# FaspDevTeam/faspsolver

Measured on AMD Instinct MI355X. Metric: AMG-PCG solve DOF/s (3D 7-pt Poisson 256^3, classical AMG V(1,1) w-Jacobi + PCG, rtol 1e-8), higher is better.
Workload: dtype f64

## Files before the change

### faspsolver_amd/__init__.py

```python
import ctypes as C
import os
import subprocess

import numpy as np

from . import _types as T
from ._types import *

_HERE = os.path.dirname(os.path.abspath(__file__))
LIB_PATH = os.environ.get("FASP_HIP_LIB") or os.path.join(_HERE, "libfasp_hip.so")
_lib = None

EXPORTS = [
    "fasp_param_amg_init", "fasp_param_solver_init", "fasp_solver_dcsr_krylov_amg",
    "fasp_blas_dcsr_mxv", "fasp_blas_dcsr_aAxpy", "fasp_blas_darray_dotprod",
    "fasp_blas_darray_norm2", "fasp_blas_darray_norminf", "fasp_blas_darray_axpy",
    "fasp_blas_darray_axpby", "fasp_smoother_dcsr_jacobi",
    "fasp_blas_dbsr_mxv", "fasp_blas_dbsr_aAxpy", "fasp_dbsr_getdiaginv", "fasp_smoother_dbsr_jacobi1",
    "fasp_solver_dbsr_pcg", "fasp_solver_dbsr_pbcgs", "fasp_solver_dbsr_pgmres", "fasp_solver_dbsr_pvgmres",
    "fasp_solver_dbsr_pvfgmres", "fasp_hip_bsr_precond_setup", "fasp_hip_bsr_precond_fct", "fasp_hip_bsr_precond_free",
    "fasp_hip_param_input", "fasp_fwrapper_dcsr_krylov_amg_", "fasp_dcsrvec_read2", "fasp_dvec_read",
    "fasp_dbsr_read", "fasp_dcoo_read", "fasp_dcoo_read1", "fasp_dcoo_shift_read", "fasp_dmtx_read", "fasp_dmtxsym_read", "fasp_dvec_write", "fasp_dcsr_write_coo", "fasp_dcsrvec_write2", "fasp_fwrapper_dcsr_amg_", "fasp_fwrapper_dbsr_krylov_amg_", "fasp_hip_free_bsr", "fasp_hip_comm_selftest", "fasp_hip_amg_kernel_info", "fasp_hip_coarse_kernel_info", "fasp_hip_bsr_coarse_kernel_info", "fasp_hip_coding_selftest", "fasp_solver_amg", "fasp_solver_famg", "fasp_hip_amg_solve", "fasp_precond_diag", "fasp_precond_dbsr_diag", "fasp_solver_dcsr_itsolver", "fasp_solver_dcsr_krylov", "fasp_solver_dcsr_krylov_diag", "fasp_solver_dbsr_itsolver", "fasp_solver_dbsr_krylov", "fasp_solver_dbsr_krylov_diag", "fasp_hip_mxv_csr", "fasp_hip_mxv_bsr", "fasp_solver_matfree_init", "fasp_solver_pcg", "fasp_solver_pbcgs", "fasp_solver_pgcg", "fasp_solver_pminres", "fasp_solver_pgmres", "fasp_solver_pvgmres", "fasp_solver_pvfgmres", "fasp_solver_itsolver", "fasp_solver_krylov", "fasp_solver_dcsr_pcg", "fasp_solver_dcsr_pminres", "fasp_solver_dcsr_pgcg", "fasp_solver_dcsr_pgcr", "fasp_solver_dcsr_pbcgs", "fasp_solver_dcsr_pgmres", "fasp_solver_dcsr_pvgmres",
    "fasp_solver_dcsr_pvfgmres", "fasp_hip_precond_setup", "fasp_hip_precond_fct", "fasp_hip_precond_free",
    "fasp_hip_time_bsr_mxv", "fasp_solver_dbsr_krylov_amg", "fasp_hip_bsr_amg_create", "fasp_hip_bsr_amg_create_host",
# ... 1 lines not shown
    "fasp_hip_bsr_amg_get_diaginv", "fasp_hip_bsr_solve",
    "fasp_hip_set_device", "fasp_hip_device_count", "fasp_hip_device_identity", "fasp_hip_available",
    "fasp_hip_amg_create", "fasp_hip_amg_create_host", "fasp_hip_amg_upload",
    "fasp_hip_amg_destroy", "fasp_hip_amg_num_levels", "fasp_hip_amg_get_matrix",
    "fasp_hip_amg_get_cfmark", "fasp_hip_solve", "fasp_hip_set_rhs", "fasp_hip_set_guess",
    "fasp_hip_solve_resident", "fasp_hip_get_solution", "fasp_hip_device_synchronize",
    "fasp_hip_precond_amg",
    "fasp_hip_poisson7pt", "fasp_hip_aniso27pt", "fasp_hip_free_system", "fasp_hip_time_kernel", "fasp_hip_measure_ceilings", "fasp_hip_amg_publish", "fasp_hip_amg_attach", "fasp_hip_amg_unpublish",
    "fasp_precond_setup", "fasp_precond_amg", "fasp_precond_famg", "fasp_precond_amli", "fasp_precond_namli", "fasp_amg_data_create", "fasp_amg_data_free", "fasp_param_amg_to_prec", "fasp_param_prec_to_amg", "fasp_mem_free", "fasp_mem_calloc", "fasp_dvec_alloc", "fasp_dvec_set", "fasp_dvec_free", "fasp_dvec_create", "fasp_dcsr_create", "fasp_dcsr_free", "fasp_smoother_dcsr_gs", "fasp_smoother_dcsr_sor", "fasp_smoother_dcsr_L1diag",
    "fasp_hip_tune", "fasp_hip_comm_unique_id", "fasp_hip_comm_init", "fasp_hip_comm_finalize",
    "fasp_hip_comm_rank", "fasp_hip_comm_size", "fasp_hip_version", "fasp_hip_comm_init_shm",
    "fasp_hip_dist_plan", "fasp_hip_dist_level_info", "fasp_hip_dist_get_matrix",
    "fasp_hip_dist_get_list",
    "fasp_blas_dcsr_vmv", "fasp_blas_dcsr_mxv_agg", "fasp_blas_dcsr_aAxpy_agg", "fasp_blas_darray_ax",
    "fasp_blas_darray_axpyz", "fasp_blas_darray_norm1", "fasp_darray_cp", "fasp_darray_set", "fasp_dvec_isnan",
    "fasp_hip_time_matrix", "fasp_hip_bsr_dist_info", "fasp_hip_seq_schedule_selftest", "fasp_hip_seq_chain_selftest", "fasp_hip_cluster_order", "fasp_hip_permute_csr", "fasp_hip_comm_init_ipc", "fasp_hip_comm_stats", "fasp_hip_comm_timing", "fasp_hip_estream_selftest", "fasp_hip_sell_selftest", "fasp_hip_csr_plan", "fasp_hip_level_op", "fasp_hip_matrix_op", "fasp_hip_matrix_traits",
    "fasp_param_ilu_init", "fasp_ilu_data_create", "fasp_ilu_data_free", "fasp_mem_iludata_check", "fasp_ilu_dcsr_setup",
    "fasp_precond_ilu", "fasp_precond_ilu_forward", "fasp_precond_ilu_backward", "fasp_solver_dcsr_krylov_ilu",
    "fasp_solver_dcsr_krylov_ilu_M", "fasp_smoother_dcsr_ilu", "fasp_fwrapper_dcsr_krylov_ilu_",
    "fasp_hip_ilu_resident_count", "fasp_hip_ilu_time",
    "fasp_ilu_dbsr_setup", "fasp_precond_dbsr_ilu", "fasp_solver_dbsr_krylov_ilu", "fasp_smoother_dbsr_ilu",
    "fasp_fwrapper_dbsr_krylov_ilu_",
    "fasp_hip_bsr_amg_get_ilu", "fasp_hip_bsr_amg_ilu_info", "fasp_hip_bsr_amg_ilu_smooth_time",
    "fasp_hip_bsr_sweep", "fasp_hip_csr_sweep",
    "fasp_blas_dcsr_rap", "fasp_hip_dcsr_rap", "fasp_hip_rap_info", "fasp_hip_rap_device_count", "fasp_hip_rap_time",
    "fasp_dstr_create", "fasp_dstr_alloc", "fasp_dstr_free", "fasp_dstr_cp", "fasp_format_dstr_dcsr", "fasp_dstr_read",
    "fasp_blas_dstr_aAxpy", "fasp_blas_dstr_mxv", "fasp_precond_dstr_diag", "fasp_solver_dstr_pcg", "fasp_solver_dstr_pbcgs",
    "fasp_solver_dstr_pminres", "fasp_solver_dstr_pgmres", "fasp_solver_dstr_pvgmres", "fasp_solver_dstr_itsolver",
    "fasp_solver_dstr_krylov", "fasp_solver_dstr_krylov_diag", "fasp_hip_mxv_str", "fasp_hip_str_form", "fasp_hip_time_str_mxv",
    "fasp_ilu_dstr_setup0", "fasp_ilu_dstr_setup1", "fasp_precond_dstr_ilu0", "fasp_precond_dstr_ilu1", "fasp_solver_dstr_krylov_ilu",
    "fasp_hip_str_ilu_form", "fasp_hip_str_ilu_apply", "fasp_hip_time_str_ilu",
# ... 674 lines not shown
```

### faspsolver_amd/csrc/device_csr.hip.h

```cpp

struct DevCSR {
    int     row = 0, col = 0, nnz = 0;
    int*    ia  = nullptr;
    int*    ja  = nullptr;
    double* val = nullptr;
    int*    dpos = nullptr;
    bool    dup_diag = false;
    bool    sorted = false;
    int     lanes = 8;
    int     kind = 0;
    int     tile_rows = 256;
    int     wrows = 64, wcap = 512;
    unsigned char* code = nullptr;
    int*    rowbase = nullptr;
    int*    doff = nullptr;
    double* dval = nullptr;
    unsigned short* pat = nullptr;
    int*    pstart = nullptr;
    int*    plen = nullptr;
    int*    poff = nullptr;
    double* pval = nullptr;
    int     npat = 0, npent = 0;
    unsigned short* ja16 = nullptr;
    int*            jbase = nullptr;
// ... 5 lines not shown
    int*    tcols = nullptr;
    long long ntcols = 0;
    const int* bridge = nullptr;
    double*    bscratch = nullptr;
    int        bridge_dir = 0;
    int*       es_tab = nullptr;
    unsigned short* es_ja16 = nullptr;
    double*    es_part = nullptr;
    int        es_W = 0, es_nc = 0;
    unsigned*      sell_code = nullptr;
    int*           sell_meta = nullptr;
    unsigned char* sell_rlen = nullptr;
    double*        sell_tab = nullptr;
    int            sell_nv = 0, sell_obits = 0, sell_nslice = 0;
    long long      sell_slots = 0;
    void    release()
    {
        if (sell_code) (void)hipFree(sell_code);
        if (sell_meta) (void)hipFree(sell_meta);
        if (sell_rlen) (void)hipFree(sell_rlen);
        if (sell_tab) (void)hipFree(sell_tab);
        sell_code = nullptr; sell_meta = nullptr; sell_rlen = nullptr; sell_tab = nullptr; sell_nv = sell_obits = sell_nslice = 0; sell_slots = 0;
        if (es_tab) (void)hipFree(es_tab);
        if (es_part) (void)hipFree(es_part);
        if (es_ja16) (void)hipFree(es_ja16);
        es_tab = nullptr; es_part = nullptr; es_ja16 = nullptr; es_W = es_nc = 0;
        if (bscratch) (void)hipFree(bscratch);
        bscratch = nullptr; bridge = nullptr; bridge_dir = 0;
        if (lja16) (void)hipFree(lja16);
        if (tptr) (void)hipFree(tptr);
        if (tcols) (void)hipFree(tcols);
        lja16 = nullptr; tptr = nullptr; tcols = nullptr;
// ... 786 lines not shown
    std::vector<int> meta(2 * ns + 1);
    std::copy(S.sptr.begin(), S.sptr.end(), meta.begin());
    std::copy(S.sbase.begin(), S.sbase.end(), meta.begin() + (long)ns + 1);
    HIPCK(hipMalloc(&D.sell_code, sizeof(unsigned) * (size_t)std::max<long long>(S.slots, 1)));
    HIPCK(hipMalloc(&D.sell_meta, sizeof(int) * meta.size()));
    HIPCK(hipMalloc(&D.sell_rlen, (size_t)H.row));
    HIPCK(hipMalloc(&D.sell_tab, sizeof(double) * (size_t)S.nv));
    HIPCK(hipMemcpy(D.sell_code, S.code.data(), sizeof(unsigned) * (size_t)S.slots, hipMemcpyHostToDevice));
    HIPCK(hipMemcpy(D.sell_meta, meta.data(), sizeof(int) * meta.size(), hipMemcpyHostToDevice));
    HIPCK(hipMemcpy(D.sell_rlen, S.rlen.data(), (size_t)H.row, hipMemcpyHostToDevice));
    HIPCK(hipMemcpy(D.sell_tab, S.tab.data(), sizeof(double) * (size_t)S.nv, hipMemcpyHostToDevice));
    D.sell_nv = S.nv; D.sell_obits = S.obits; D.sell_nslice = S.nslice; D.sell_slots = S.slots;
    return FASP_SUCCESS;
}

static int upload_csr(const HostCSR& H, DevCSR& D)
{
    D.row = H.row; D.col = H.col; D.nnz = H.nnz;
    HIPCK(hipMalloc(&D.ia, sizeof(int) * ((size_t)H.row + 1)));
    HIPCK(hipMalloc(&D.ja, sizeof(int) * std::max<size_t>(H.nnz, 1)));
    HIPCK(hipMalloc(&D.val, sizeof(double) * (std::max<size_t>(H.nnz, 1) + 2)));
    HIPCK(hipMemsetAsync(D.val + std::max<size_t>(H.nnz, 1), 0, sizeof(double) * 2, g_ctx.stream));
    HIPCK(hipMemcpyAsync(D.ia, H.ia.data(), sizeof(int) * ((size_t)H.row + 1), hipMemcpyHostToDevice, g_ctx.stream));
    pick_kernel(D);
    auto upload_plain = [&]() -> int {
        HIPCK(hipMemcpyAsync(D.ja, H.ja.data(), sizeof(int) * (size_t)H.nnz, hipMemcpyHostToDevice, g_ctx.stream));
        HIPCK(hipMemcpyAsync(D.val, H.val.data(), sizeof(double) * (size_t)H.nnz, hipMemcpyHostToDevice, g_ctx.stream));
        return 0;
    };
    if (compress_enabled() && H.nnz >= 4096 && (double)H.nnz <= 48.0 * H.row) {
        Buf<unsigned short> pat; Buf<int> prb;
        std::vector<int> pstart, plen, poff; std::vector<double> pval;
        static const bool rowpat_on = !(std::getenv("FASP_HIP_ROWPAT") && std::atoi(std::getenv("FASP_HIP_ROWPAT")) == 0);
        if (rowpat_on && build_rowpat(H, pat, pstart, plen, poff, pval, prb)) {
            D.npat = (int)pstart.size(); D.npent = (int)poff.size();
            HIPCK(hipMalloc(&D.pat, sizeof(unsigned short) * ((size_t)H.row + 2)));
            HIPCK(hipMalloc(&D.pstart, sizeof(int) * pstart.size()));
            HIPCK(hipMalloc(&D.plen, sizeof(int) * plen.size()));
            HIPCK(hipMemcpy(D.plen, plen.data(), sizeof(int) * plen.size(), hipMemcpyHostToDevice));
// ... 101 lines not shown
        lap("row sort");
        HIPCK(hipMemcpy(D.ja, sj.data(), sizeof(int) * (size_t)H.nnz, hipMemcpyHostToDevice));
        HIPCK(hipMemcpy(D.val, sv.data(), sizeof(double) * (size_t)H.nnz, hipMemcpyHostToDevice));
        lap("memcpy");
        if (square && D.kind == 2) {
            HIPCK(hipMalloc(&D.dpos, sizeof(int) * (size_t)std::max(H.row, 1)));
            HIPCK(hipMemcpy(D.dpos, dp.data(), sizeof(int) * (size_t)H.row, hipMemcpyHostToDevice));
        }
        D.sorted = true;
        if (upload_ja16(D, H.ia.data(), sj.data()) < 0) return ERROR_ALLOC_MEM;
        return build_estream(H.ia.data(), H.row, H.nnz, D);
    }
    if (upload_plain() < 0) return ERROR_ALLOC_MEM;
    if (D.kind == 2 && !g_oneshot_upload && build_xtile(H, D) < 0) return ERROR_ALLOC_MEM;
    if (D.kind == 2 && compress_enabled() && upload_sell(H, D) < 0) return ERROR_ALLOC_MEM;
    if (upload_ja16(D, H.ia.data(), H.ja.data()) < 0) return ERROR_ALLOC_MEM;
    return build_estream(H.ia.data(), H.row, H.nnz, D);
}

struct Tuning { int ilu_smooth_fused = 1, gen2 = 2, ws2_bpc = 3, maxgrid = -1, xcd = 16, nt = 1, kind = -1, lanes = -1, wrows = -1, wcap = -1, compress = 1, rpl = -1, lds_tab = 1, xcd_pat = 64, spcg_batch = 16, small_lds = 1, ja16 = 1, spcg_fused = 1, spcg_grid = 0, spcg_persist = 1, split_rows = 0, gs_multicolor = 0, seq_flow = 1, seq_strip_kb = 0, seq_jobs = 1, seq_spine = 1, seq_grid = 0, seq_chain = 1, seq_chain_n1 = 0, seq_chain_grid = 0, seq_chain_ref = 0, seq_test_hang = 0, seq_rest_lanes = 0, local_square = 1, fuse_zr = 1, fuse_presmooth = 1, seq_lanes = 0, xtile = 1, rp5_max = 45, rp_bpc = 5, rp_xcd = -1, rp_strip = 2, spcg_test_hang = 0, small_onewave = 4, lazy_coarse = 1, rp_stream = -1, renumber = 1, renumber_chunk = 262144, pcg_dev_beta = 1, spcg_spec = 1, ev_every = 4, pcg_fold = 1, seq_chain_touch = 8, seq_chain_touch_t1 = 1, seq_zero_skip = 1, estream = 1, es_dbg = 0, ilu_form = -1, str_ilu_form = -1, str_ilu_wgs = 0, str_sweep_form = -1, str_sweep_wgs = 0, sell = 1; };
static Tuning g_tune;

template <class K>
static int resident_blocks_per_cu(K kernel)
{
    static std::vector<std::pair<const void*, int>> cache;
    const void* key = reinterpret_cast<const void*>(kernel);
    for (const auto& e : cache)
        if (e.first == key) return e.second;
    int nb = 0;
// ... 9 lines not shown
    int cap = (blocks_per_cu > 0 ? std::min(blocks_per_cu, resident_blocks_per_cu(kernel)) : resident_blocks_per_cu(kernel)) * g_ctx.num_cu;
    if (g_tune.maxgrid > 0) cap = g_tune.maxgrid;
    cap = std::min(cap, MAXGRID);
    int grid = std::min(cap, ntiles);
    grid = std::max(8, (grid + 7) / 8 * 8);
    hipLaunchKernelGGL(kernel, dim3(grid), dim3(BLOCK), 0, g_ctx.stream, a);
    return grid;
}

enum CsrKernel : int {
    CK_ROWS_2 = 0, CK_ROWS_4, CK_ROWS_8, CK_ROWS_16, CK_ROWS_32, CK_ROWS_64,
    CK_WSTREAM_64_512, CK_WSTREAM_64_1024, CK_WSTREAM_32_512, CK_WSTREAM_32_1024,
    CK_ROWPAT_0_1, CK_ROWPAT_0_2, CK_ROWPAT_1_1, CK_ROWPAT_1_2, CK_ROWPAT_2_1, CK_ROWPAT_2_2,
    CK_DICT8_8, CK_DICT8_16, CK_DICT8_24,
    CK_ESTREAM_4, CK_ESTREAM_8, CK_ESTREAM_16, CK_ESTREAM_32,
    CK_ROWPAT4, CK_ROWPAT5, CK_LSTREAM, CK_XTILE, CK_SELL, CK_WSTREAM2
};
struct CsrPlan {
    CsrKernel kernel;
    int    family;
    int    tile_rows;
    int    bpc;
    int    xcd_map;
    int    tpp;
    int    nt;
    bool   ja16, jbase;
    bool   fused_zr;
    double bytes;
};
static CsrPlan plan_csr(const DevCSR& M, int op, bool windowed, bool want_partials, int rows = -1)
{
// ... 31 lines not shown
    }
    else if (pair && g_tune.gen2 >= 2 && M.rowbase && !jac && op != OP_L1DIAG && (double)M.nnz <= 0.1 * g_tune.rp5_max * M.row) {
        p.kernel = CK_ROWPAT5; p.family = 9; p.tile_rows = 2 * BLOCK; p.bpc = 5;
        p.xcd_map = ntiles() >= 8 * 64 ? -1 : 16;
        if (g_tune.rp_strip >= 2) strips();
    }
    else if (kind == 5) {
        const int rpl = g_tune.rpl > 0 ? g_tune.rpl : 1;
        const bool lds = M.npat <= 512 && M.npent <= 2048 && g_tune.lds_tab != 0;
        const int T = !lds ? 0 : M.npat <= 64 && M.npent <= 512 && g_tune.lds_tab != 3 ? 2 : 1;
        p.kernel = CsrKernel(CK_ROWPAT_0_1 + 2 * T + (rpl != 1)); p.family = 5; p.tile_rows = BLOCK * rpl;
        if (g_tune.xcd_pat != 0) p.xcd_map = g_tune.xcd_pat;
        if (g_tune.xcd_pat == 64 && g_tune.rp_strip >= 2) strips();
    }
    else if (kind == 4) { p.kernel = avg <= 8.5 ? CK_DICT8_8 : avg <= 20.0 ? CK_DICT8_16 : CK_DICT8_24; p.family = 4; }
    else if (lstream_ok) { p.kernel = CK_LSTREAM; p.family = 7; p.bpc = 4; p.fused_zr = jac && want_partials; }
    else if (kind == 2 && g_tune.gen2 >= 2 && w64) {
        if (g_tune.xtile && M.lja16) {
            p.kernel = CK_XTILE; p.family = 10; p.bpc = 3;
            p.bytes = 10.0 * M.nnz + ptr_bytes + 4.0 * M.ntcols + 4.0 * ((M.row + 63) / 64 + 1.0);
        }
        else if (M.sell_code && g_tune.compress && g_tune.sell) {
            p.kernel = CK_SELL; p.family = 11; p.tile_rows = SELL_BLOCK;
            p.bytes = 4.0 * (double)M.sell_slots + 1.0 * M.row + 4.0 * (2.0 * M.sell_nslice + 1.0) + 8.0 * M.sell_nv;
        }
        else { p.kernel = CK_WSTREAM2; p.family = 8; p.bpc = g_tune.ws2_bpc; }
        p.fused_zr = jac && want_partials;
    }
    else if (kind == 2) {
        p.kernel = w64 ? CK_WSTREAM_64_512 : wrows == 64 ? CK_WSTREAM_64_1024 : wrows == 32 && wcap == 512 ? CK_WSTREAM_32_512 : CK_WSTREAM_32_1024; p.family = 2;
// ... 30 lines not shown
    int nb = 0;
    for (const auto& e : cache)
        if (e.first == lds) nb = e.second;
    if (nb == 0) {
        if (hipOccupancyMaxActiveBlocksPerMultiprocessor(&nb, k_csr_sell<OP>, SELL_BLOCK, lds) != hipSuccess || nb < 1) nb = 1;
        nb = std::min(nb, 2);
        cache.emplace_back(lds, nb);
    }
    int cap = nb * g_ctx.num_cu;
    if (g_tune.maxgrid > 0) cap = g_tune.maxgrid;
    cap = std::min(cap, MAXGRID);
    int grid = std::min(cap, a.ntiles);
    grid = std::max(8, (grid + 7) / 8 * 8);
    hipLaunchKernelGGL(k_csr_sell<OP>, dim3(grid), dim3(SELL_BLOCK), lds, g_ctx.stream, a);
    return grid;
}

template <int OP>
static int launch_rowpat5(CsrArgs& a)
{
    if constexpr (OP == OP_JACOBI || OP == OP_L1DIAG) { (void)a; return 0; }
    else return launch_persistent(k_csr_rowpat5<OP>, a.ntiles, a, 5);
}

constexpr int WIN_ALIGN = DIST_WIN_ALIGN;
struct RowWin { int lo = 0, hi = -1, goff = 0; };

__global__ __launch_bounds__(BLOCK) void k_bridge_gather(int n, const int* __restrict__ perm, const double* __restrict__ s, double* __restrict__ y,
                                                         double* __restrict__ zx, const double* __restrict__ zdiag, double zomega)
{
// ... 78 lines not shown
        case CK_ROWPAT_0_1: PERSIST(k_csr_rowpat<OP, 0, 1>);
        case CK_ROWPAT_0_2: PERSIST(k_csr_rowpat<OP, 0, 2>);
        case CK_ROWPAT_1_1: PERSIST(k_csr_rowpat<OP, 1, 1>);
        case CK_ROWPAT_1_2: PERSIST(k_csr_rowpat<OP, 1, 2>);
        case CK_ROWPAT_2_1: PERSIST(k_csr_rowpat<OP, 2, 1>);
        case CK_ROWPAT_2_2: PERSIST(k_csr_rowpat<OP, 2, 2>);
        case CK_DICT8_8:  PERSIST(k_csr_dict8<OP, 8>);
        case CK_DICT8_16: PERSIST(k_csr_dict8<OP, 16>);
        case CK_DICT8_24: PERSIST(k_csr_dict8<OP, 24>);
        case CK_ROWPAT4:  PERSIST(k_csr_rowpat4<OP>);
        case CK_ROWPAT5:  return launch_rowpat5<OP>(a);
        case CK_LSTREAM:  PERSIST(k_csr_lstream<OP, 512>);
        case CK_XTILE:    PERSIST(k_csr_xtile<OP>);
        case CK_SELL:     return launch_sell<OP>(M, a);
        case CK_WSTREAM2: PERSIST(k_csr_wstream2<OP>);
        default: break;
    }
#undef PERSIST
    const int W = M.es_W, nc = M.es_nc, lanes = 4 << (p.kernel - CK_ESTREAM_4);
    a.es_wc = M.es_tab; a.es_centry = a.es_wc + W + 1; a.es_crow = a.es_centry + nc + 1; a.es_hw0 = a.es_crow + nc + 1; a.es_np = a.es_hw0 + W;
    a.es_part = M.es_part; a.es_cnt = reinterpret_cast<unsigned*>(M.es_part + 2 * (size_t)W);
    a.es_cbase = M.es_ja16 ? a.es_np + W : nullptr; a.es_ja16 = M.es_ja16;
    static bool attr_set = false;
#define ES_ATTR(LL) (void)hipFuncSetAttribute(reinterpret_cast<const void*>(k_csr_estream<LL, OP>), hipFuncAttributeMaxDynamicSharedMemorySize, ES_LDS_BYTES)
    if (!attr_set) { ES_ATTR(32); ES_ATTR(16); ES_ATTR(8); ES_ATTR(4); attr_set = true; }
#undef ES_ATTR
#define ES_LAUNCH(LL) hipLaunchKernelGGL((k_csr_estream<LL, OP>), dim3(W / 4), dim3(BLOCK), ES_LDS_BYTES, g_ctx.stream, a)
#ifdef FASP_LAB_DEBUG
    if (OP == OP_MXV && g_tune.es_dbg) {
#define ES_DBG(LL, DD) do { (void)hipFuncSetAttribute(reinterpret_cast<const void*>(k_csr_estream<LL, OP_MXV, DD>), hipFuncAttributeMaxDynamicSharedMemorySize, ES_LDS_BYTES); hipLaunchKernelGGL((k_csr_estream<LL, OP_MXV, DD>), dim3(W / 4), dim3(BLOCK), ES_LDS_BYTES, g_ctx.stream, a); } while (0)
// ... 88 lines not shown
```

### faspsolver_amd/csrc/kernels.hip.h

```cpp
#pragma once

#include <hip/hip_runtime.h>

namespace fasp {

constexpr int BLOCK   = 256;
constexpr int MAXGRID = 2048;

enum RowOp : int {
    OP_MXV = 0,
    OP_RESID,
    OP_ADD,
    OP_SUB,
    OP_AXPY,
    OP_JACOBI,
    OP_L1DIAG,
    OP_MXV_DOT
};

struct CsrArgs {
    int           nrow;
    const int*    ia;
    const int*    ja;
    const double* val;
// ... 36 lines not shown
    const int*    es_wc;
    const int*    es_centry;
    const int*    es_crow;
    const int*    es_hw0;
    const int*    es_np;
    const int*    es_cbase;
    const unsigned short* es_ja16;
    double*       es_part;
    unsigned*     es_cnt;
    const unsigned*      sell_code;
    const int*           sell_sptr;
    const int*           sell_sbase;
    const unsigned char* sell_rlen;
    const double*        sell_tab;
    int                  sell_nv, sell_obits;
};

__device__ __forceinline__ void zx_store(const CsrArgs& a, int r, double s)
{
    if (a.zx) {
        const double di = a.zdiag[r];
        a.zx[r] = (fabs(di) > 1e-20) ? (1 - a.zomega) * 0.0 + a.zomega * s / di : 0.0;
    }
}

__device__ __forceinline__ double l1_or_jacobi_f(const CsrArgs& a, int r, double t, double d, double xi)
{
    if (a.mark) return a.mark[r] == 0 ? xi + a.omega * t / d : xi;
    return (fabs(d) > 1e-20) ? xi + t / d : xi;
}
// ... 1053 lines not shown
```

### faspsolver_amd/csrc/solver.hip

```cpp
#include <hip/hip_runtime.h>

#include <fcntl.h>
#include <omp.h>
#include <sys/mman.h>
#include <sys/stat.h>
#include <unistd.h>

#include <algorithm>
#include <cfloat>
#include <cmath>
#include <cstdio>
#include <cstdlib>
#include <cstring>
#include <functional>
#include <condition_variable>
#include <memory>
#include <mutex>
#include <string>
#include <thread>
#include <vector>

#include "fasp_comm.h"
#include "fasp_internal.h"
#include "krylov_ws.h"
#include "kernels.hip.h"
#include "kernels2.hip.h"
#include "kernels3.hip.h"
#include "kernels4.hip.h"
#include "small_solvers.hip.h"
#include "seq_split.hip.h"
#include "seq_chain.hip.h"

namespace fasp {

#define HIPCK(expr)                                                                        \
    do {                                                                                   \
        hipError_t e_ = (expr);                                                            \
        if (e_ != hipSuccess) {                                                            \
            std::fprintf(stderr, "### ERROR: fasp_hip: %s failed: %s [%s:%d]\n", #expr,    \
                         hipGetErrorString(e_), __FILE__, __LINE__);                       \
            return ERROR_MISC;                                                             \
        }                                                                                  \
    } while (0)
// ... 2042 lines not shown
    else if (!std::strcmp(key, "seq_spine")) g_tune.seq_spine = value;
    else if (!std::strcmp(key, "seq_partition")) g_seq_partition = value;
    else if (!std::strcmp(key, "fuse_zr")) g_tune.fuse_zr = value;
    else if (!std::strcmp(key, "fuse_presmooth")) g_tune.fuse_presmooth = value;
    else if (!std::strcmp(key, "seq_lanes")) g_tune.seq_lanes = value;
    else if (!std::strcmp(key, "lazy_coarse")) g_tune.lazy_coarse = value;
    else if (!std::strcmp(key, "xtile")) g_tune.xtile = value;
    else if (!std::strcmp(key, "rp5_max")) g_tune.rp5_max = value;
    else if (!std::strcmp(key, "rp_bpc")) g_tune.rp_bpc = value;
    else if (!std::strcmp(key, "rp_stream")) g_tune.rp_stream = value;
    else if (!std::strcmp(key, "renumber")) g_tune.renumber = value;
    else if (!std::strcmp(key, "renumber_chunk")) g_tune.renumber_chunk = value;
    else if (!std::strcmp(key, "time_cold")) g_time_cold = value;
    else if (!std::strcmp(key, "estream")) g_tune.estream = value;
    else if (!std::strcmp(key, "sell")) g_tune.sell = value;
    else if (!std::strcmp(key, "es_dbg")) g_tune.es_dbg = value;
    else if (!std::strcmp(key, "pcg_dev_beta")) g_tune.pcg_dev_beta = value;
    else if (!std::strcmp(key, "seq_chain_touch")) g_tune.seq_chain_touch = value;
    else if (!std::strcmp(key, "seq_chain_touch_t1")) g_tune.seq_chain_touch_t1 = value;
    else if (!std::strcmp(key, "seq_zero_skip")) g_tune.seq_zero_skip = value;
    else if (!std::strcmp(key, "pcg_fold")) g_tune.pcg_fold = value;
    else if (!std::strcmp(key, "spcg_spec")) g_tune.spcg_spec = value;
    else if (!std::strcmp(key, "ev_every")) g_tune.ev_every = value;
    else if (!std::strcmp(key, "rp_xcd")) g_tune.rp_xcd = value;
    else if (!std::strcmp(key, "rp_strip")) g_tune.rp_strip = value;
    else if (!std::strcmp(key, "host_parallel_min")) g_parallel_min_nnz = value;
    else if (!std::strcmp(key, "rap_form")) g_rap_form = value;
    else if (!std::strcmp(key, "rap_arena_kb")) g_rap_arena_kb = value;
    else if (!std::strcmp(key, "device_rap")) g_device_rap = value;
    else if (!std::strcmp(key, "lanes")) g_tune.lanes = value;
// ... 9 lines not shown
    HostCSR M;
    M.row = A->row; M.col = A->col; M.nnz = A->nnz;
    M.ia.view(A->IA, (size_t)A->row + 1); M.ja.view(A->JA, (size_t)std::max(A->nnz, 1)); M.val.view(A->val, (size_t)std::max(A->nnz, 1));
    SellHost S;
    int why = 0;
    const bool ok = build_sell(M, S, cap_percent > 0 ? cap_percent : SELL_CAP_PERCENT, &why);
    info[0] = ok ? 1 : 0; info[1] = why; info[2] = S.nv; info[3] = S.vbits; info[4] = S.obits; info[5] = S.nslice;
    info[6] = ok ? (int)std::min<long long>(S.slots / 64, 0x7fffffff) : 0; info[7] = SELL_MAXV;
    if (bytes) *bytes = ok ? S.bytes(M.row) : 0.0;
    if (!ok) return FASP_SUCCESS;
    if (ia_out && ja_out && val_out) sell_decode_host(S, M.row, ia_out, ja_out, val_out);
    if (x && y) sell_mxv_host(S, M.row, x, y);
    return FASP_SUCCESS;
}

int fasp_hip_csr_plan(const int* traits, int op, int windowed, int want_partials, int* plan, double* bytes)
{
    FASP_ENTRY();
    if (!traits || !plan || op < OP_MXV || op > OP_MXV_DOT) return ERROR_INPUT_PAR;
    static double dummy[1];
    const int* t = traits;
    auto flag = [&](int i) -> void* { return t[i] ? dummy : nullptr; };
    DevCSR M;
    M.row = t[0]; M.col = t[1]; M.nnz = t[2]; M.kind = t[3]; M.lanes = t[4]; M.wrows = t[5]; M.wcap = t[6]; M.nxrows = t[7]; M.plane = t[8];
    M.npat = t[9]; M.npent = t[10]; M.sell_nv = t[11]; M.sell_nslice = t[12]; M.sell_slots = t[13]; M.ntcols = t[14]; M.es_W = t[15]; M.es_nc = t[16];
    M.code = (unsigned char*)flag(17); M.pat = (unsigned short*)flag(18); M.rowbase = (int*)flag(19); M.dpos = (int*)flag(20); M.dup_diag = t[21] != 0;
    M.ja16 = (unsigned short*)flag(22); M.jbase = (int*)flag(23); M.lja16 = (unsigned short*)flag(24); M.sell_code = (unsigned*)flag(25);
    M.es_tab = (int*)flag(26); M.es_ja16 = (unsigned short*)flag(27);
    const CsrPlan p = plan_csr(M, op, windowed || g_tune.split_rows > 0, want_partials != 0);
    const int out[11] = {(int)p.kernel, p.family, p.tile_rows, p.bpc, p.xcd_map, p.tpp, p.nt, p.ja16, p.jbase, p.fused_zr, kernel_family(M, nullptr)};
    std::copy(out, out + 11, plan);
    if (bytes) *bytes = p.bytes;
    return FASP_SUCCESS;
}

int fasp_hip_estream_selftest(const int* ia, int nrow, int nnz, int per_wave, int wmax, int* info)
{
    if (!ia || nrow < 1 || nnz < 1 || per_wave < 8 || wmax < 32) return ERROR_INPUT_PAR;
    return estream_selftest_host(ia, nrow, nnz, per_wave, wmax, info);
}

int fasp_hip_measure_ceilings(double* out, size_t bytes, int reps)
{
// ... 245 lines not shown
```

### include/fasp_hip_dev.h

```cpp
#ifndef FASP_HIP_DEV_H
#define FASP_HIP_DEV_H
#include "fasp_hip.h"
#ifdef __cplusplus
extern "C" {
#endif

double fasp_hip_time_kernel(fasp_hip_amg* h, int kind, int level, int reps);
double fasp_hip_time_matrix(const dCSRmat* A, int op, int reps, int* kind_out);
double fasp_hip_seq_schedule_selftest(const dCSRmat* A, const int* seq, int ns, int strip_kb, int lanes, int spine, int* info);
int fasp_hip_cluster_order(const dCSRmat* A, int chunk, int* order);
int fasp_hip_permute_csr(const dCSRmat* A, const int* rperm, const int* cinv, int* ia, int* ja, double* val);
double fasp_hip_seq_chain_selftest(const dCSRmat* A, const int* seq, int ns, int n1_blocks, int form, double w, int* info, double* out_u);
int fasp_hip_measure_ceilings(double* out, size_t bytes, int reps);

int    fasp_hip_ilu_resident_count(void);
double fasp_hip_ilu_time(ILU_data* iludata, int which, int reps, double* info);
int    fasp_hip_bsr_amg_get_ilu(const fasp_hip_amg_bsr* h, int level, ILU_data* view);
int    fasp_hip_bsr_amg_ilu_info(const fasp_hip_amg_bsr* h, int level, double info[6]);
double fasp_hip_bsr_amg_ilu_smooth_time(fasp_hip_amg_bsr* h, int level, int reps);

int    fasp_hip_dcsr_rap(const dCSRmat* R, const dCSRmat* A, const dCSRmat* P, dCSRmat* RAP);
int    fasp_hip_rap_info(int info[4]);
long   fasp_hip_rap_device_count(void);
double fasp_hip_rap_time(const dCSRmat* R, const dCSRmat* A, const dCSRmat* P, int where, int reps);

int fasp_hip_tune(const char* key, int value);
int fasp_hip_coarse_kernel_info(const fasp_hip_amg* h, int* info);
int fasp_hip_bsr_coarse_kernel_info(const fasp_hip_amg_bsr* h, int* info);

int fasp_hip_comm_stats(double* out8, int reset);
int fasp_hip_comm_timing(int on);

int fasp_hip_dist_plan(fasp_hip_amg* h, int rank, int nranks, int min_rows);
int fasp_hip_dist_level_info(const fasp_hip_amg* h, int level, int* info);
int fasp_hip_dist_get_matrix(const fasp_hip_amg* h, int level, int which, dCSRmat* view);
int fasp_hip_dist_get_list(const fasp_hip_amg* h, int level, int which, ivector* view);
int  fasp_hip_estream_selftest(const int* ia, int nrow, int nnz, int per_wave, int wmax, int* info);
int  fasp_hip_csr_plan(const int* traits, int op, int windowed, int want_partials, int* plan, double* bytes);
int  fasp_hip_sell_selftest(const dCSRmat* A, int cap_percent, int* info, double* bytes, int* ia_out, int* ja_out, double* val_out, const double* x, double* y);
int  fasp_hip_level_op(fasp_hip_amg* h, int level, int which, int op, const double* x, const double* b, double* y, double* y2, double scalar, double* red);
int  fasp_hip_matrix_op(const dCSRmat* A, int op, const double* x, const double* b, double* y, double* y2, double scalar, double* red, int* kind_out);
int  fasp_hip_matrix_traits(const dCSRmat* A, int* traits);
int  fasp_hip_bsr_sweep(const dBSRmat* A, const double* b, double* u, const double* diaginv, int descend, int sor, double w, int* nlevels);
int  fasp_hip_csr_sweep(const dCSRmat* A, const int* seq, int ns, int form, double w, int zero_start, const double* b, double* u, int* info);
int  fasp_hip_str_form(const dSTRmat* A);
double fasp_hip_time_str_mxv(const dSTRmat* A, int reps);
int    fasp_hip_str_ilu_form(const dSTRmat* LU, int lfil);
int    fasp_hip_str_ilu_apply(const dSTRmat* LU, int lfil, const double* r, double* z);
double fasp_hip_time_str_ilu(const dSTRmat* LU, int lfil, int reps);
int    fasp_hip_str_sweep(const dSTRmat* A, int kind, int order, const int* mark, double weight, const double* diaginv, const double* b,
                          double* u, int nsweeps, int* info);
int    fasp_hip_str_sweep_form(const dSTRmat* A, int order, const int* mark);
int    fasp_hip_str_sweep_levels(const dSTRmat* A, int order, const int* mark, int* visit, int* level, int cap);
// ... 11 lines not shown
```

Before: 472.8 million.

## Add value-dictionary compressed CSR kernel for transfer operators

Adds a "vcode" compressed CSR format that packs each entry into one 32-bit word: an index into a small table of distinct values plus a column offset from a per-64-row tile base. A new persistent kernel stages the packed words in LDS with software double-buffering and uses a wave scan to locate row spans. It applies to rectangular transfer operators (kind 2, non-Jacobi, non-windowed) and aims to cut SpMV memory traffic from 12 bytes per nonzero to about 4. The cost is extra setup time for host-side hashing and encoding, a fallback when the matrix has too many distinct values, and more plan-selection complexity.

```diff
diff --git a/faspsolver_amd/__init__.py b/faspsolver_amd/__init__.py
--- a/faspsolver_amd/__init__.py
+++ b/faspsolver_amd/__init__.py
@@ -39,7 +39,7 @@
     "fasp_hip_dist_get_list",
     "fasp_blas_dcsr_vmv", "fasp_blas_dcsr_mxv_agg", "fasp_blas_dcsr_aAxpy_agg", "fasp_blas_darray_ax",
     "fasp_blas_darray_axpyz", "fasp_blas_darray_norm1", "fasp_darray_cp", "fasp_darray_set", "fasp_dvec_isnan",
-    "fasp_hip_time_matrix", "fasp_hip_bsr_dist_info", "fasp_hip_seq_schedule_selftest", "fasp_hip_seq_chain_selftest", "fasp_hip_cluster_order", "fasp_hip_permute_csr", "fasp_hip_comm_init_ipc", "fasp_hip_comm_stats", "fasp_hip_comm_timing", "fasp_hip_estream_selftest", "fasp_hip_sell_selftest", "fasp_hip_csr_plan", "fasp_hip_level_op", "fasp_hip_matrix_op", "fasp_hip_matrix_traits",
+    "fasp_hip_time_matrix", "fasp_hip_bsr_dist_info", "fasp_hip_seq_schedule_selftest", "fasp_hip_seq_chain_selftest", "fasp_hip_cluster_order", "fasp_hip_permute_csr", "fasp_hip_comm_init_ipc", "fasp_hip_comm_stats", "fasp_hip_comm_timing", "fasp_hip_estream_selftest", "fasp_hip_sell_selftest", "fasp_hip_vcode_selftest", "fasp_hip_csr_plan", "fasp_hip_csr_plan_n", "fasp_hip_level_op", "fasp_hip_matrix_op", "fasp_hip_matrix_traits",
     "fasp_param_ilu_init", "fasp_ilu_data_create", "fasp_ilu_data_free", "fasp_mem_iludata_check", "fasp_ilu_dcsr_setup",
     "fasp_precond_ilu", "fasp_precond_ilu_forward", "fasp_precond_ilu_backward", "fasp_solver_dcsr_krylov_ilu",
     "fasp_solver_dcsr_krylov_ilu_M", "fasp_smoother_dcsr_ilu", "fasp_fwrapper_dcsr_krylov_ilu_",
diff --git a/faspsolver_amd/csrc/device_csr.hip.h b/faspsolver_amd/csrc/device_csr.hip.h
--- a/faspsolver_amd/csrc/device_csr.hip.h
+++ b/faspsolver_amd/csrc/device_csr.hip.h
@@ -43,8 +43,18 @@
     double*        sell_tab = nullptr;
     int            sell_nv = 0, sell_obits = 0, sell_nslice = 0;
     long long      sell_slots = 0;
+    unsigned*      vc_code = nullptr;
+    int*           vc_meta = nullptr;
+    unsigned char* vc_rlen = nullptr;
+    double*        vc_tab = nullptr;
+    int            vc_nv = 0, vc_obits = 0, vc_ntile = 0;
     void    release()
     {
+        if (vc_code) (void)hipFree(vc_code);
+        if (vc_meta) (void)hipFree(vc_meta);
+        if (vc_rlen) (void)hipFree(vc_rlen);
+        if (vc_tab) (void)hipFree(vc_tab);
+        vc_code = nullptr; vc_meta = nullptr; vc_rlen = nullptr; vc_tab = nullptr; vc_nv = vc_obits = vc_ntile = 0;
         if (sell_code) (void)hipFree(sell_code);
         if (sell_meta) (void)hipFree(sell_meta);
         if (sell_rlen) (void)hipFree(sell_rlen);
@@ -861,6 +871,189 @@
     return FASP_SUCCESS;
 }
 
+struct VcodeHost {
+    int ntile = 0, nv = 0, vbits = 0, obits = 0;
+    std::vector<int> meta;
+    std::vector<unsigned char> rlen;
+    std::vector<double> tab;
+    Buf<unsigned> code;
+    double bytes(int nrow, int nnz) const { return 4.0 * nnz + 1.0 * nrow + 8.0 * ntile + 8.0 * nv; }
+};
+static bool build_vcode(const HostCSR& M, VcodeHost& S, int* why_not)
+{
+    int dummy = 0;
+    int& why = why_not ? *why_not : dummy;
+    why = 1;
+    const int n = M.row;
+    if (n <= 0 || M.nnz <= 0 || (double)M.nnz > 7.6 * n) return false;
+    if ((long long)M.col >= (1ll << 28)) return false;
+    const int nt64 = (n + 63) / 64;
+    S.ntile = nt64;
+    S.rlen.assign((size_t)n, 0);
+    int toolong = 0;
+#pragma omp parallel for schedule(static) reduction(+ : toolong)
+    for (int r = 0; r < n; ++r) {
+        const int len = M.ia[r + 1] - M.ia[r];
+        if (len > 255) ++toolong; else S.rlen[(size_t)r] = (unsigned char)len;
+    }
+    if (toolong) { why = 2; return false; }
+    constexpr int VSLOTS = 4096;
+    struct VSet {
+        unsigned long long key[VSLOTS];
+        long long cnt[VSLOTS];
+        int id[VSLOTS];
+        int n = 0;
+        VSet() { for (int s = 0; s < VSLOTS; ++s) { key[s] = 0ull; cnt[s] = 0; id[s] = -1; } }
+        static unsigned slot_of(unsigned long long b) { return (unsigned)((b * 0x9E3779B97F4A7C15ull) >> 52); }
+        bool add(unsigned long long b, long long c)
+        {
+            unsigned s = slot_of(b);
+            for (;;) {
+                if (cnt[s] == 0) {
+                    if (n >= VC_MAXV) return false;
+                    key[s] = b; cnt[s] = c; ++n;
+                    return true;
+                }
+                if (key[s] == b) { cnt[s] += c; return true; }
+                s = (s + 1) & (VSLOTS - 1);
+            }
+        }
+        int slot(unsigned long long b) const
+        {
+            unsigned s = slot_of(b);
+            for (;;) {
+                if (cnt[s] == 0) return -1;
+                if (key[s] == b) return (int)s;
+                s = (s + 1) & (VSLOTS - 1);
+            }
+        }
+    };
+    auto bits_of = [](double v) { unsigned long long b; std::memcpy(&b, &v, 8); return b; };
+    const int nthr = std::max(1, std::min(omp_get_max_threads(), n / 4096 + 1));
+    std::vector<VSet*> local((size_t)nthr, nullptr);
+    bool fail = false;
+#pragma omp parallel num_threads(nthr)
+    {
+        VSet* T = new VSet();
+        local[(size_t)omp_get_thread_num()] = T;
+#pragma omp for schedule(static)
+        for (int r = 0; r < n; ++r) {
+            if (fail) continue;
+            for (int k = M.ia[r]; k < M.ia[r + 1]; ++k)
+                if (!T->add(bits_of(M.val[k]), 1)) { fail = true; break; }
+        }
+    }
+    std::unique_ptr<VSet> Gs(new VSet());
+    for (VSet* T : local) {
+        if (T && !fail)
+            for (int s = 0; s < VSLOTS && !fail; ++s)
+                if (T->cnt[s] && !Gs->add(T->key[s], T->cnt[s])) fail = true;
+        delete T;
+    }
+    if (fail) { why = 4; return false; }
+    std::vector<std::pair<long long, unsigned long long>> order;
+    for (int s = 0; s < VSLOTS; ++s)
+        if (Gs->cnt[s]) order.emplace_back(-Gs->cnt[s], Gs->key[s]);
+    std::sort(order.begin(), order.end());
+    S.nv = (int)order.size();
+    S.tab.resize(order.size());
+    for (size_t i = 0; i < order.size(); ++i) std::memcpy(&S.tab[i], &order[i].second, 8);
+    for (size_t i = 0; i < order.size(); ++i) Gs->id[Gs->slot(order[i].second)] = (int)i;
+    S.vbits = 0;
+    while ((1ll << S.vbits) < S.nv) ++S.vbits;
+    S.meta.assign(2 * (size_t)nt64, 0);
+    int maxoff = 0;
+#pragma omp parallel for schedule(static) reduction(max : maxoff)
+    for (int t = 0; t < nt64; ++t) {
+        const int k0 = M.ia[t * 64], k1 = M.ia[std::min(n, t * 64 + 64)];
+        S.meta[2 * (size_t)t] = k0;
+        if (k1 <= k0) continue;
+        int lo = M.ja[k0], hi = lo;
+        for (int k = k0 + 1; k < k1; ++k) { lo = std::min(lo, M.ja[k]); hi = std::max(hi, M.ja[k]); }
+        S.meta[2 * (size_t)t + 1] = lo;
+        maxoff = std::max(maxoff, hi - lo);
+    }
+    S.obits = 1;
+    while ((1ll << S.obits) <= maxoff) ++S.obits;
+    if (S.vbits + S.obits > 32) { why = 5; return false; }
+    S.code.alloc((size_t)M.nnz);
+    bool lost = false;
+    const VSet& GS = *Gs;
+#pragma omp parallel for schedule(static)
+    for (int t = 0; t < nt64; ++t) {
+        const int k0 = M.ia[t * 64], k1 = M.ia[std::min(n, t * 64 + 64)], base = S.meta[2 * (size_t)t + 1];
+        for (int k = k0; k < k1; ++k) {
+            const int sl = GS.slot(bits_of(M.val[k]));
+            if (sl < 0) { lost = true; continue; }
+            S.code[k] = ((unsigned)GS.id[sl] << S.obits) | (unsigned)(M.ja[k] - base);
+        }
+    }
+    if (lost) { why = 4; return false; }
+    why = 0;
+    return true;
+}
+
+static void vcode_mxv_host(const VcodeHost& S, int nrow, const double* x, double* y)
+{
+    const unsigned omask = (1u << S.obits) - 1u;
+    for (int t = 0; t < S.ntile; ++t) {
+        int k = S.meta[2 * (size_t)t];
+        const int base = S.meta[2 * (size_t)t + 1];
+        for (int r = t * 64; r < std::min(nrow, t * 64 + 64); ++r) {
+            double acc = 0.0;
+            for (int e = 0; e < (int)S.rlen[(size_t)r]; ++e, ++k) {
+                const unsigned c = S.code[(size_t)k];
+                acc = acc + S.tab[c >> S.obits] * x[base + (int)(c & omask)];
+            }
+            y[r] = acc;
+        }
+    }
+}
+static void vcode_decode_host(const VcodeHost& S, int nrow, int* ia, int* ja, double* val)
+{
+    const unsigned omask = (1u << S.obits) - 1u;
+    ia[0] = 0;
+    for (int r = 0; r < nrow; ++r) ia[r + 1] = ia[r] + (int)S.rlen[(size_t)r];
+    for (int t = 0; t < S.ntile; ++t) {
+        int k = S.meta[2 * (size_t)t];
+        const int base = S.meta[2 * (size_t)t + 1];
+        for (int r = t * 64; r < std::min(nrow, t * 64 + 64); ++r)
+            for (int e = 0; e < (int)S.rlen[(size_t)r]; ++e, ++k) {
+                const unsigned c = S.code[(size_t)k];
+                ja[ia[r] + e] = base + (int)(c & omask);
+                val[ia[r] + e] = S.tab[c >> S.obits];
+            }
+    }
+}
+
+static int g_vcode = 1;
+static int g_vc_bpc = 8;
+constexpr int VC_MIN_NNZ = 4096;
+static int upload_vcode(const HostCSR& H, DevCSR& D)
+{
+    if (H.nnz < VC_MIN_NNZ && g_vcode < 2) return FASP_SUCCESS;
+    static const bool timing = std::getenv("FASP_HIP_SETUP_TIMING") != nullptr;
+    const double t0 = wall_seconds();
+    VcodeHost S;
+    int why = 0;
+    const bool ok = build_vcode(H, S, &why);
+    if (timing) std::printf("        [vcode %d x %d, %d nnz] %s (%d) %d values, %d + %d bits, %.3f s\n", H.row, H.col, H.nnz,
+                            ok ? "coded" : "not coded", why, S.nv, S.vbits, S.obits, wall_seconds() - t0);
+    if (!ok) return FASP_SUCCESS;
+    const size_t nw = (size_t)H.nnz + 4;
+    HIPCK(hipMalloc(&D.vc_code, sizeof(unsigned) * nw));
+    HIPCK(hipMalloc(&D.vc_meta, sizeof(int) * S.meta.size()));
+    HIPCK(hipMalloc(&D.vc_rlen, (size_t)H.row));
+    HIPCK(hipMalloc(&D.vc_tab, sizeof(double) * (size_t)S.nv));
+    HIPCK(hipMemset(D.vc_code + H.nnz, 0, sizeof(unsigned) * 4));
+    HIPCK(hipMemcpy(D.vc_code, S.code.data(), sizeof(unsigned) * (size_t)H.nnz, hipMemcpyHostToDevice));
+    HIPCK(hipMemcpy(D.vc_meta, S.meta.data(), sizeof(int) * S.meta.size(), hipMemcpyHostToDevice));
+    HIPCK(hipMemcpy(D.vc_rlen, S.rlen.data(), (size_t)H.row, hipMemcpyHostToDevice));
+    HIPCK(hipMemcpy(D.vc_tab, S.tab.data(), sizeof(double) * (size_t)S.nv, hipMemcpyHostToDevice));
+    D.vc_nv = S.nv; D.vc_obits = S.obits; D.vc_ntile = S.ntile;
+    return FASP_SUCCESS;
+}
+
 static int upload_csr(const HostCSR& H, DevCSR& D)
 {
     D.row = H.row; D.col = H.col; D.nnz = H.nnz;
@@ -870,6 +1063,7 @@
     HIPCK(hipMemsetAsync(D.val + std::max<size_t>(H.nnz, 1), 0, sizeof(double) * 2, g_ctx.stream));
     HIPCK(hipMemcpyAsync(D.ia, H.ia.data(), sizeof(int) * ((size_t)H.row + 1), hipMemcpyHostToDevice, g_ctx.stream));
     pick_kernel(D);
+    if (g_vcode >= 2 && D.kind == 0 && H.row != H.col && (double)H.nnz <= 7.6 * H.row) D.kind = 2;
     auto upload_plain = [&]() -> int {
         HIPCK(hipMemcpyAsync(D.ja, H.ja.data(), sizeof(int) * (size_t)H.nnz, hipMemcpyHostToDevice, g_ctx.stream));
         HIPCK(hipMemcpyAsync(D.val, H.val.data(), sizeof(double) * (size_t)H.nnz, hipMemcpyHostToDevice, g_ctx.stream));
@@ -1001,6 +1195,7 @@
     if (upload_plain() < 0) return ERROR_ALLOC_MEM;
     if (D.kind == 2 && !g_oneshot_upload && build_xtile(H, D) < 0) return ERROR_ALLOC_MEM;
     if (D.kind == 2 && compress_enabled() && upload_sell(H, D) < 0) return ERROR_ALLOC_MEM;
+    if (D.kind == 2 && compress_enabled() && g_vcode && upload_vcode(H, D) < 0) return ERROR_ALLOC_MEM;
     if (upload_ja16(D, H.ia.data(), H.ja.data()) < 0) return ERROR_ALLOC_MEM;
     return build_estream(H.ia.data(), H.row, H.nnz, D);
 }
@@ -1040,7 +1235,8 @@
     CK_ROWPAT_0_1, CK_ROWPAT_0_2, CK_ROWPAT_1_1, CK_ROWPAT_1_2, CK_ROWPAT_2_1, CK_ROWPAT_2_2,
     CK_DICT8_8, CK_DICT8_16, CK_DICT8_24,
     CK_ESTREAM_4, CK_ESTREAM_8, CK_ESTREAM_16, CK_ESTREAM_32,
-    CK_ROWPAT4, CK_ROWPAT5, CK_LSTREAM, CK_XTILE, CK_SELL, CK_WSTREAM2
+    CK_ROWPAT4, CK_ROWPAT5, CK_LSTREAM, CK_XTILE, CK_SELL, CK_WSTREAM2,
+    CK_VCODE
 };
 struct CsrPlan {
     CsrKernel kernel;
@@ -1102,6 +1298,10 @@
         if (g_tune.xcd_pat == 64 && g_tune.rp_strip >= 2) strips();
     }
     else if (kind == 4) { p.kernel = avg <= 8.5 ? CK_DICT8_8 : avg <= 20.0 ? CK_DICT8_16 : CK_DICT8_24; p.family = 4; }
+    else if (lstream_ok && M.vc_code && g_tune.compress && g_vcode && !windowed && !jac && op != OP_L1DIAG) {
+        p.kernel = CK_VCODE; p.family = 12; p.bpc = g_vc_bpc;
+        p.bytes = 4.0 * M.nnz + 1.0 * M.row + 8.0 * M.vc_ntile + 8.0 * M.vc_nv;
+    }
     else if (lstream_ok) { p.kernel = CK_LSTREAM; p.family = 7; p.bpc = 4; p.fused_zr = jac && want_partials; }
     else if (kind == 2 && g_tune.gen2 >= 2 && w64) {
         if (g_tune.xtile && M.lja16) {
@@ -1162,6 +1362,16 @@
     grid = std::max(8, (grid + 7) / 8 * 8);
     hipLaunchKernelGGL(k_csr_sell<OP>, dim3(grid), dim3(SELL_BLOCK), lds, g_ctx.stream, a);
     return grid;
+}
+
+template <int OP>
+static int launch_vcode(const DevCSR& M, CsrArgs& a, int bpc)
+{
+    if constexpr (OP == OP_JACOBI || OP == OP_L1DIAG) { (void)M; (void)a; (void)bpc; return 0; }
+    else {
+        a.vc_code = M.vc_code; a.vc_meta = M.vc_meta; a.vc_rlen = M.vc_rlen; a.vc_tab = M.vc_tab; a.vc_nv = M.vc_nv; a.vc_obits = M.vc_obits;
+        return launch_persistent(k_csr_vcode<OP>, a.ntiles, a, bpc);
+    }
 }
 
 template <int OP>
@@ -1270,6 +1480,7 @@
         case CK_XTILE:    PERSIST(k_csr_xtile<OP>);
         case CK_SELL:     return launch_sell<OP>(M, a);
         case CK_WSTREAM2: PERSIST(k_csr_wstream2<OP>);
+        case CK_VCODE:    return launch_vcode<OP>(M, a, p.bpc);
         default: break;
     }
 #undef PERSIST
diff --git a/faspsolver_amd/csrc/kernels.hip.h b/faspsolver_amd/csrc/kernels.hip.h
--- a/faspsolver_amd/csrc/kernels.hip.h
+++ b/faspsolver_amd/csrc/kernels.hip.h
@@ -74,6 +74,11 @@
     const unsigned char* sell_rlen;
     const double*        sell_tab;
     int                  sell_nv, sell_obits;
+    const unsigned*      vc_code;
+    const int*           vc_meta;
+    const unsigned char* vc_rlen;
+    const double*        vc_tab;
+    int                  vc_nv, vc_obits;
 };
 
 __device__ __forceinline__ void zx_store(const CsrArgs& a, int r, double s)
diff --git a/faspsolver_amd/csrc/kernels5.hip.h b/faspsolver_amd/csrc/kernels5.hip.h
--- /dev/null
+++ b/faspsolver_amd/csrc/kernels5.hip.h
@@ -0,0 +1,176 @@
+#pragma once
+
+#include "kernels4.hip.h"
+
+namespace fasp {
+
+constexpr int VC_MAXV = 1024;
+constexpr int VC_CAP  = 512;
+
+__device__ __forceinline__ int wave_scan_incl(int v, int lane)
+{
+#pragma unroll
+    for (int d = 1; d < 64; d <<= 1) {
+        const int t = __shfl_up(v, d, 64);
+        if (lane >= d) v += t;
+    }
+    return v;
+}
+
+template <int OP>
+__global__ __launch_bounds__(BLOCK) void k_csr_vcode(CsrArgs a)
+{
+    static_assert(OP != OP_JACOBI && OP != OP_L1DIAG, "transfer-operator kernel");
+    if (a.stop && *a.stop) return;
+    constexpr int NJ = VC_CAP / 256;
+    __shared__ __attribute__((aligned(16))) double   tab[VC_MAXV];
+    __shared__ __attribute__((aligned(16))) unsigned sw_all[4 * VC_CAP];
+    __shared__ double red[4];
+    const int lane = threadIdx.x & 63, wave = __builtin_amdgcn_readfirstlane(threadIdx.x >> 6);
+    for (int i = threadIdx.x; i < a.vc_nv; i += BLOCK) tab[i] = a.vc_tab[i];
+    __syncthreads();
+    unsigned* sw = sw_all + wave * VC_CAP;
+    const int      obits = a.vc_obits;
+    const unsigned omask = (1u << obits) - 1u;
+    const int vmax = tile_vmax(a);
+    const int G = gridDim.x;
+    double dotacc = 0.0;
+
+    auto advance = [&](int& v, int& r0, int& nr) {
+        for (;;) {
+            r0 = -1; nr = 0;
+            if (v >= vmax) return;
+            const int t = tile_of(a, v);
+            v += G;
+            if (t >= a.ntiles) continue;
+            const int rr = (t + a.tile0) * BLOCK + wave * 64;
+            if (rr >= a.nrow) continue;
+            r0 = rr; nr = min(64, a.nrow - rr);
+            return;
+        }
+    };
+    auto load_meta = [&](int r0, int nr, int& len, int& first, int& base) {
+        len = first = base = 0;
+        if (r0 < 0) return;
+        if (lane < nr) len = a.vc_rlen[r0 + lane];
+        const int t = r0 >> 6;
+        first = a.vc_meta[2 * t]; base = a.vc_meta[2 * t + 1];
+    };
+    auto span = [&](int r0, int len, int first, int& s0, int& k1, int& kb) {
+        s0 = k1 = kb = 0;
+        if (r0 < 0) return;
+        const int incl = wave_scan_incl(len, lane);
+        s0 = first & ~3;
+        k1 = first + __builtin_amdgcn_readlane(incl, 63);
+        kb = first + incl - len;
+    };
+    u32x4_t q[NJ];
+    auto stage_load = [&](int s0, int k1) {
+        const int n = k1 - s0;
+        if (n > VC_CAP) return;
+        const u32x4_t* p = reinterpret_cast<const u32x4_t*>(a.vc_code + s0);
+#pragma unroll
+        for (int j = 0; j < NJ; ++j)
+            if ((lane + 64 * j) * 4 < n) q[j] = __builtin_nontemporal_load(p + lane + 64 * j);
+    };
+    auto stage_store = [&](int s0, int k1) {
+        const int n = k1 - s0;
+        if (n > VC_CAP) return;
+#pragma unroll
+        for (int j = 0; j < NJ; ++j)
+            if ((lane + 64 * j) * 4 < n) reinterpret_cast<u32x4_t*>(sw)[lane + 64 * j] = q[j];
+    };
+
+    int v = blockIdx.x;
+    int r0A, nrA, lenA, firstA, baseA, s0A, k1A, kbA;
+    int r0B, nrB, lenB, firstB, baseB, s0B, k1B, kbB;
+    advance(v, r0A, nrA);
+    load_meta(r0A, nrA, lenA, firstA, baseA);
+    advance(v, r0B, nrB);
+    load_meta(r0B, nrB, lenB, firstB, baseB);
+    span(r0A, lenA, firstA, s0A, k1A, kbA);
+    if (r0A >= 0) { stage_load(s0A, k1A); stage_store(s0A, k1A); }
+    wave_order();
+
+    while (r0A >= 0) {
+        const bool fit = (k1A - s0A) <= VC_CAP;
+        const int  r = r0A + lane;
+        const int  len = lenA;
+        const int  o = kbA - s0A;
+        double acc = 0.0;
+        double pre = 0.0;
+        if (lane < nrA) {
+            if (OP == OP_ADD || OP == OP_SUB || OP == OP_AXPY) pre = a.y[r];
+            else if (OP == OP_RESID) pre = a.b[r];
+            else if (OP == OP_MXV_DOT) pre = a.dotv[r];
+        }
+
+        unsigned w[8];
+        int      c[8];
+        double   xv[8];
+        if (fit) {
+#pragma unroll
+            for (int u = 0; u < 8; ++u) {
+                const unsigned ww = sw[(u < len) ? o + u : 0];
+                w[u] = (u < len) ? ww : 0u;
+                c[u] = (u < len) ? baseA + (int)(ww & omask) : 0;
+            }
+#pragma unroll
+            for (int u = 0; u < 8; ++u) xv[u] = __any(u < len) ? a.x[c[u]] : 0.0;
+        }
+
+        span(r0B, lenB, firstB, s0B, k1B, kbB);
+        if (r0B >= 0) stage_load(s0B, k1B);
+        int r0C, nrC, lenC, firstC, baseC;
+        advance(v, r0C, nrC);
+        load_meta(r0C, nrC, lenC, firstC, baseC);
+
+        if (fit) {
+#pragma unroll
+            for (int u = 0; u < 8; ++u) {
+                const double pr = tab[w[u] >> obits] * xv[u];
+                acc = (u < len) ? acc + pr : acc;
+            }
+            for (int j = 8; __any(j < len); j += 8) {
+#pragma unroll
+                for (int u = 0; u < 8; ++u) {
+                    const unsigned ww = sw[(j + u < len) ? o + j + u : 0];
+                    w[u] = (j + u < len) ? ww : 0u;
+                    c[u] = (j + u < len) ? baseA + (int)(ww & omask) : 0;
+                }
+#pragma unroll
+                for (int u = 0; u < 8; ++u) xv[u] = a.x[c[u]];
+#pragma unroll
+                for (int u = 0; u < 8; ++u) {
+                    const double pr = tab[w[u] >> obits] * xv[u];
+                    acc = (j + u < len) ? acc + pr : acc;
+                }
+            }
+        } else {
+            for (int k = kbA; k < kbA + len; ++k) {
+                const unsigned ww = a.vc_code[k];
+                acc += tab[ww >> obits] * a.x[baseA + (int)(ww & omask)];
+            }
+        }
+        if (lane < nrA) {
+            if (OP == OP_MXV) row_epilogue<OP>(a, r, acc, dotacc);
+            else if (OP == OP_RESID) a.y[r] = pre - acc;
+            else if (OP == OP_ADD) a.y[r] = pre + acc;
+            else if (OP == OP_SUB) a.y[r] = pre - acc;
+            else if (OP == OP_AXPY) a.y[r] = pre + acc * a.alpha;
+            else { a.y[r] = acc; dotacc += acc * pre; }
+        }
+
+        wave_order();
+        if (r0B >= 0) stage_store(s0B, k1B);
+        wave_order();
+        r0A = r0B; nrA = nrB; lenA = lenB; firstA = firstB; baseA = baseB; s0A = s0B; k1A = k1B; kbA = kbB;
+        r0B = r0C; nrB = nrC; lenB = lenC; firstB = firstC; baseB = baseC;
+    }
+    if (OP == OP_MXV_DOT) {
+        const double tot = block_sum(dotacc, red);
+        if (threadIdx.x == 0) a.partials[blockIdx.x] = tot;
+    }
+}
+
+}
diff --git a/faspsolver_amd/csrc/solver.hip b/faspsolver_amd/csrc/solver.hip
--- a/faspsolver_amd/csrc/solver.hip
+++ b/faspsolver_amd/csrc/solver.hip
@@ -27,6 +27,7 @@
 #include "kernels2.hip.h"
 #include "kernels3.hip.h"
 #include "kernels4.hip.h"
+#include "kernels5.hip.h"
 #include "small_solvers.hip.h"
 #include "seq_split.hip.h"
 #include "seq_chain.hip.h"
@@ -2099,6 +2100,8 @@
     else if (!std::strcmp(key, "time_cold")) g_time_cold = value;
     else if (!std::strcmp(key, "estream")) g_tune.estream = value;
     else if (!std::strcmp(key, "sell")) g_tune.sell = value;
+    else if (!std::strcmp(key, "vcode")) g_vcode = value;
+    else if (!std::strcmp(key, "vc_bpc")) g_vc_bpc = value;
     else if (!std::strcmp(key, "es_dbg")) g_tune.es_dbg = value;
     else if (!std::strcmp(key, "pcg_dev_beta")) g_tune.pcg_dev_beta = value;
     else if (!std::strcmp(key, "seq_chain_touch")) g_tune.seq_chain_touch = value;
@@ -2138,10 +2141,33 @@
     return FASP_SUCCESS;
 }
 
+int fasp_hip_vcode_selftest(const dCSRmat* A, int* info, double* bytes, int* ia_out, int* ja_out, double* val_out, const double* x, double* y, int* meta_out)
+{
+    if (!A || !info || A->row < 0 || A->nnz < 0) return ERROR_INPUT_PAR;
+    HostCSR M;
+    M.row = A->row; M.col = A->col; M.nnz = A->nnz;
+    M.ia.view(A->IA, (size_t)A->row + 1); M.ja.view(A->JA, (size_t)std::max(A->nnz, 1)); M.val.view(A->val, (size_t)std::max(A->nnz, 1));
+    VcodeHost S;
+    int why = 0;
+    const bool ok = build_vcode(M, S, &why);
+    info[0] = ok ? 1 : 0; info[1] = why; info[2] = S.nv; info[3] = S.vbits; info[4] = S.obits; info[5] = S.ntile; info[6] = VC_MAXV;
+    info[7] = ok ? (int)S.code.n : 0; info[8] = ok ? (int)S.rlen.size() : 0; info[9] = ok ? (int)S.meta.size() : 0;
+    if (bytes) *bytes = ok ? S.bytes(M.row, M.nnz) : 0.0;
+    if (!ok) return FASP_SUCCESS;
+    if (ia_out && ja_out && val_out) vcode_decode_host(S, M.row, ia_out, ja_out, val_out);
+    if (x && y) vcode_mxv_host(S, M.row, x, y);
+    if (meta_out) std::copy(S.meta.begin(), S.meta.end(), meta_out);
+    return FASP_SUCCESS;
+}
+
 int fasp_hip_csr_plan(const int* traits, int op, int windowed, int want_partials, int* plan, double* bytes)
 {
-    FASP_ENTRY();
-    if (!traits || !plan || op < OP_MXV || op > OP_MXV_DOT) return ERROR_INPUT_PAR;
+    return fasp_hip_csr_plan_n(traits, 28, op, windowed, want_partials, plan, bytes);
+}
+int fasp_hip_csr_plan_n(const int* traits, int ntraits, int op, int windowed, int want_partials, int* plan, double* bytes)
+{
+    FASP_ENTRY();
+    if (!traits || ntraits < 28 || !plan || op < OP_MXV || op > OP_MXV_DOT) return ERROR_INPUT_PAR;
     static double dummy[1];
     const int* t = traits;
     auto flag = [&](int i) -> void* { return t[i] ? dummy : nullptr; };
@@ -2151,6 +2177,9 @@
     M.code = (unsigned char*)flag(17); M.pat = (unsigned short*)flag(18); M.rowbase = (int*)flag(19); M.dpos = (int*)flag(20); M.dup_diag = t[21] != 0;
     M.ja16 = (unsigned short*)flag(22); M.jbase = (int*)flag(23); M.lja16 = (unsigned short*)flag(24); M.sell_code = (unsigned*)flag(25);
     M.es_tab = (int*)flag(26); M.es_ja16 = (unsigned short*)flag(27);
+    if (ntraits > 28) M.vc_code = (unsigned*)flag(28);
+    if (ntraits > 29) M.vc_nv = t[29];
+    if (ntraits > 30) M.vc_ntile = t[30];
     const CsrPlan p = plan_csr(M, op, windowed || g_tune.split_rows > 0, want_partials != 0);
     const int out[11] = {(int)p.kernel, p.family, p.tile_rows, p.bpc, p.xcd_map, p.tpp, p.nt, p.ja16, p.jbase, p.fused_zr, kernel_family(M, nullptr)};
     std::copy(out, out + 11, plan);
diff --git a/include/fasp_hip_dev.h b/include/fasp_hip_dev.h
--- a/include/fasp_hip_dev.h
+++ b/include/fasp_hip_dev.h
@@ -37,6 +37,8 @@
 int fasp_hip_dist_get_list(const fasp_hip_amg* h, int level, int which, ivector* view);
 int  fasp_hip_estream_selftest(const int* ia, int nrow, int nnz, int per_wave, int wmax, int* info);
 int  fasp_hip_csr_plan(const int* traits, int op, int windowed, int want_partials, int* plan, double* bytes);
+int  fasp_hip_csr_plan_n(const int* traits, int ntraits, int op, int windowed, int want_partials, int* plan, double* bytes);
+int  fasp_hip_vcode_selftest(const dCSRmat* A, int* info, double* bytes, int* ia_out, int* ja_out, double* val_out, const double* x, double* y, int* meta_out);
 int  fasp_hip_sell_selftest(const dCSRmat* A, int cap_percent, int* info, double* bytes, int* ia_out, int* ja_out, double* val_out, const double* x, double* y);
 int  fasp_hip_level_op(fasp_hip_amg* h, int level, int which, int op, const double* x, const double* b, double* y, double* y2, double scalar, double* red);
 int  fasp_hip_matrix_op(const dCSRmat* A, int op, const double* x, const double* b, double* y, double* y2, double scalar, double* red, int* kind_out);
```

New measurement: 480.0 million, median of 6. 1.5% higher.
